# fchchen/omni-recall-rag

Measured on AMD Instinct MI355X. Metric: queries/sec at top-k=10 over N x 3072-d chunks; score delta vs C# reference in `parity`, higher is better.
Workload: dtype i8 screen + f32*f32->f64 exact re-score; 1 GPU; C3: 10000000 chunks x 3072-d fp32 on one GPU, batch=256 queries per step, top-k=10, full hybrid (cosine+keyword+recency), candidate_limit=corpus; corpus_rows=10000000

## Files before the change

### omni-recall-rag_amd/csrc/orr_api.hip

```cpp
#include <hip/hip_runtime.h>

#include <algorithm>
#include <cmath>
#include <cstdarg>
#include <cstdio>
#include <chrono>
#include <pthread.h>
#include <dlfcn.h>
#include <atomic>
#include <condition_variable>
#include <functional>
#include <cstring>
#include <limits>
#include <mutex>
#include <shared_mutex>
#include <deque>
#include <new>
#include <numeric>
#include <string>
#include <string_view>
#include <thread>
#include <unordered_map>
#include <vector>

// ... 106 lines not shown

}

struct orr_index {
    int device = 0;
    int32_t dim = 0;
    int64_t row_base = 0;
    hipStream_t stream = nullptr;
    hipStream_t stream_kw = nullptr;
    hipStream_t stream_aux = nullptr;
    hipEvent_t ev_bm_clean = nullptr;
    bool bm_clean_pending = false;
    bool kw_counters_clean = false;
    const void *kw_counters_of[2] = {nullptr, nullptr};
    hipEvent_t ev_inputs = nullptr, ev_kw_done = nullptr, ev_main_ready = nullptr, ev_range[15] = {};
    std::mutex mu;

    int64_t n_rows = 0, cap_rows = 0;
    float *d_emb = nullptr;
    int64_t *d_created = nullptr;
    int64_t *d_row_ids = nullptr;
    uint64_t *d_cstart = nullptr;
    uint32_t *d_clen = nullptr;
    uint8_t *d_pool = nullptr;
    uint64_t pool_len = 0, pool_cap = 0;
    double *d_norm_b = nullptr;
    int64_t n_tokens = 0;
    uint8_t *d_vpool = nullptr;
    uint64_t *d_vstart = nullptr;
    uint32_t *d_vlen = nullptr;
// ... 428 lines not shown
    HIP_TRY(hipGetDeviceProperties(&prop, cfg->device));
    if (strncmp(prop.gcnArchName, "gfx950", 6) != 0)
        return fail(ORR_EDEVICE, "device %d is %s; this library carries gfx950 code only", cfg->device, prop.gcnArchName);
    orr_index *idx = new (std::nothrow) orr_index();
    if (!idx) return fail(ORR_ENOMEM, "out of host memory");
    idx->device = cfg->device;
    idx->dim = cfg->dim;
    idx->row_base = cfg->row_base;
    if (hipSetDevice(idx->device) != hipSuccess || hipStreamCreateWithFlags(&idx->stream, hipStreamNonBlocking) != hipSuccess ||
        hipStreamCreateWithFlags(&idx->stream_kw, hipStreamNonBlocking) != hipSuccess ||
        hipStreamCreateWithFlags(&idx->stream_aux, hipStreamNonBlocking) != hipSuccess ||
        hipEventCreateWithFlags(&idx->ev_bm_clean, hipEventDisableTiming) != hipSuccess ||
        hipEventCreateWithFlags(&idx->ev_inputs, hipEventDisableTiming) != hipSuccess ||
        hipEventCreateWithFlags(&idx->ev_kw_done, hipEventDisableTiming) != hipSuccess ||
        hipEventCreateWithFlags(&idx->ev_main_ready, hipEventDisableTiming) != hipSuccess ||
        !create_range_events(idx->ev_range) ||
        hipEventCreateWithFlags(&idx->ev_q, hipEventDisableTiming) != hipSuccess) {
        orr_index_destroy(idx);
        return fail(ORR_EDEVICE, "cannot create streams on device %d", cfg->device);
    }
    if (cfg->capacity_rows > 0) {
        int r = ensure_row_capacity(idx, cfg->capacity_rows);
        if (r != ORR_OK) { orr_index_destroy(idx); return r; }
    }
    *out = idx;
    return ORR_OK;
}

void orr_index_destroy(orr_index *idx)
{
// ... 5 lines not shown
            LanePool::Exclusive all(&idx->lanes);
            views = idx->lanes.drain();
            idx->lanes.set_max_lanes(1);
        }
        for (orr_index *l : views) orr_index_destroy(l);
    }
    (void)hipSetDevice(idx->device);
    if (idx->stream) (void)hipStreamSynchronize(idx->stream);
    if (idx->stream_kw) (void)hipStreamSynchronize(idx->stream_kw);
    if (idx->stream_aux) (void)hipStreamSynchronize(idx->stream_aux);
    if (idx->ev_bm_clean) (void)hipEventDestroy(idx->ev_bm_clean);
    if (idx->stream_aux) (void)hipStreamDestroy(idx->stream_aux);
    if (idx->ev_inputs) (void)hipEventDestroy(idx->ev_inputs);
    if (idx->ev_kw_done) (void)hipEventDestroy(idx->ev_kw_done);
    if (idx->ev_main_ready) (void)hipEventDestroy(idx->ev_main_ready);
    for (hipEvent_t e : idx->ev_range) if (e) (void)hipEventDestroy(e);
    if (idx->stream_kw) (void)hipStreamDestroy(idx->stream_kw);
    for (auto &pe : idx->pending) { (void)hipEventDestroy(pe.start); (void)hipEventDestroy(pe.stop); }
    for (auto e : idx->event_pool) (void)hipEventDestroy(e);
    if (!idx->is_view) {
        if (idx->d_emb) (void)hipFree(idx->d_emb);
        if (idx->d_created) (void)hipFree(idx->d_created);
        if (idx->d_row_ids) (void)hipFree(idx->d_row_ids);
        if (idx->d_cstart) (void)hipFree(idx->d_cstart);
        if (idx->d_clen) (void)hipFree(idx->d_clen);
        if (idx->d_pool) (void)hipFree(idx->d_pool);
        if (idx->d_norm_b) (void)hipFree(idx->d_norm_b);
        if (idx->d_vpool) (void)hipFree(idx->d_vpool);
        if (idx->d_vstart) (void)hipFree(idx->d_vstart);
        if (idx->d_vlen) (void)hipFree(idx->d_vlen);
// ... 1309 lines not shown
    v->device = parent->device; v->dim = parent->dim; v->row_base = parent->row_base;
    v->n_rows = parent->n_rows; v->cap_rows = parent->cap_rows;
    v->d_emb = parent->d_emb; v->d_created = parent->d_created; v->d_row_ids = parent->d_row_ids; v->d_norm_b = parent->d_norm_b;
    v->n_tokens = parent->n_tokens; v->d_vpool = parent->d_vpool; v->d_vstart = parent->d_vstart; v->d_vlen = parent->d_vlen;
    v->d_post_off = parent->d_post_off; v->d_post_rows = parent->d_post_rows; v->n_postings = parent->n_postings;
    v->sealed = true;
    copy_options(parent, v);
    borrow_shadows(parent, v);
    if (hipStreamCreateWithFlags(&v->stream, hipStreamNonBlocking) != hipSuccess ||
        hipStreamCreateWithFlags(&v->stream_kw, hipStreamNonBlocking) != hipSuccess ||
        hipStreamCreateWithFlags(&v->stream_aux, hipStreamNonBlocking) != hipSuccess ||
        hipEventCreateWithFlags(&v->ev_bm_clean, hipEventDisableTiming) != hipSuccess ||
        hipEventCreateWithFlags(&v->ev_inputs, hipEventDisableTiming) != hipSuccess ||
        hipEventCreateWithFlags(&v->ev_kw_done, hipEventDisableTiming) != hipSuccess ||
        hipEventCreateWithFlags(&v->ev_main_ready, hipEventDisableTiming) != hipSuccess ||
        !create_range_events(v->ev_range) ||
        hipEventCreateWithFlags(&v->ev_q, hipEventDisableTiming) != hipSuccess) {
        v->internal_lane = true;
        orr_index_destroy(v);
        return fail(ORR_EDEVICE, "cannot create streams on device %d", parent->device);
    }
    v->internal_lane = internal;
    if (!internal) parent->user_views.fetch_add(1);
    *out = v;
    return ORR_OK;
}

int orr_index_screen_dots(orr_index *idx, int32_t B, int32_t dim, const float *q, float *out)
{
    if (!idx || !q || !out || B <= 0) return fail(ORR_EINVAL, "orr_index_screen_dots: bad argument");
// ... 32 lines not shown
    if (dim != idx->dim || dim <= 0 || dim % 128 != 0) return fail(ORR_EINVAL, "orr_index_screen_i8_dots: dim must equal the index dimension and be a multiple of 128");
    if (form > 0 && dim / 64 <= 6) return fail(ORR_EINVAL, "orr_index_screen_i8_dots: the four-wave forms need dim >= 448");
    if (idx->n_rows <= 0) return ORR_OK;
    HIP_TRY(hipSetDevice(idx->device));
    ORR_TRY(ensure_i8_shadow(idx));
    if (!idx->i8_ready) return fail(ORR_ENOMEM, "orr_index_screen_i8_dots: the int8 shadow does not fit in device memory");
    hipStream_t s = idx->stream;
    const size_t n = (size_t)idx->n_rows;
    ORR_TRY(idx->ws_q.reserve(sizeof(float) * (size_t)B * dim));
    ORR_TRY(idx->ws_q8.reserve(2 * (size_t)B * dim));
    ORR_TRY(idx->ws_q8s1.reserve(sizeof(float) * (size_t)B));
    ORR_TRY(idx->ws_q8err.reserve(2 * sizeof(double) * (size_t)B));
    ORR_TRY(idx->ws_qtiled.reserve(orr::i8_tiled_bytes(B, dim)));
    HIP_TRY(hipMemcpyAsync(idx->ws_q.p, q, sizeof(float) * (size_t)B * dim, hipMemcpyDefault, s));
    HIP_TRY(orr::launch_i8_queries(idx->ws_q.as<float>(), B, dim, idx->ws_q8.p, idx->ws_q8s1.as<float>(), idx->ws_q8err.as<double>(), s,
                                   idx->ws_q8err.as<double>() + B));
    HIP_TRY(orr::launch_i8_tile_queries(idx->ws_q8.p, B, dim, idx->ws_qtiled.p, s));
    if (out_dots) {
        ORR_TRY(idx->ws_dotf.reserve(sizeof(int32_t) * (size_t)B * n));
        HIP_TRY(hipMemsetAsync(idx->ws_dotf.p, 0xAB, sizeof(int32_t) * (size_t)B * n, s));
        ORR_TRY(idx->ws_tickets.reserve(sizeof(uint32_t) * 8 * 16));
        HIP_TRY(hipMemsetAsync(idx->ws_tickets.p, 0, sizeof(uint32_t) * 8 * 16, s));
        {
            Timed t(idx, form == 0 ? "screen_i8_dots_w8" : form == 1 ? "screen_i8_dots_w4" : "screen_i8_dots_w16",
                    1.0 * (double)n * dim + 1.0 * (double)B * dim + 4.0 * (double)B * (double)n);
            HIP_TRY(orr::launch_screen_i8_dots_raw(idx->ws_qtiled.p, B, idx->emb_i8.p, idx->n_rows, dim, idx->ws_dotf.as<int32_t>(),
                                                   idx->n_rows, form, nt_rows != 0, s, idx->ws_tickets.as<uint32_t>()));
        }
        HIP_TRY(hipMemcpyAsync(out_dots, idx->ws_dotf.p, sizeof(int32_t) * (size_t)B * n, hipMemcpyDefault, s));
    }
    if (out_iq) HIP_TRY(hipMemcpyAsync(out_iq, idx->ws_q8.p, (size_t)B * dim, hipMemcpyDefault, s));
    if (out_ie) {
// ... 217 lines not shown
        if (!on) return;
        const auto now = std::chrono::steady_clock::now();
        acc[i] += std::chrono::duration<double, std::milli>(now - last).count();
        last = now;
    }
    void done()
    {
        if (!on || ++calls % 64 != 0) return;
        fprintf(stderr, "[orr host ms/call] query_setup+cos_launch %.3f | keyword_prep+launch %.3f | norms+consts %.3f | select_launches %.3f | "
                        "wait_gpu %.3f | finish %.3f\n", acc[0] / 64, acc[1] / 64, acc[2] / 64, acc[3] / 64, acc[4] / 64, acc[5] / 64);
        for (double &x : acc) x = 0;
    }
};
thread_local HostTiming g_ht;

struct KwSide {
    orr::KwView view{nullptr, 0, nullptr, nullptr, nullptr};
    size_t bm_bytes = 0, bm_clean_before = 0;
    bool overflow_possible = false;
    uint32_t max_hits = 0;
    const uint8_t *alias = nullptr;
};

int launch_keyword_side(orr_index *idx, const BatchArgs &a, const std::vector<uint32_t> &qoff, KwSide &out)
{
    const int32_t B = a.B;
    const uint32_t t_begin = qoff[0], n_terms_total = qoff[(size_t)B] - qoff[0];
    if (n_terms_total == 0) return ORR_OK;
    {

        std::vector<std::string_view> dterms;
        dterms.reserve(n_terms_total);
        uint32_t table_size = 16;
        while (table_size < 2 * n_terms_total + 2) table_size <<= 1;
        std::vector<uint32_t> table(table_size, 0xFFFFFFFFu);
        std::vector<uint32_t> qmeta((size_t)n_terms_total + (size_t)B + 1);
// ... 183 lines not shown
            {
                Timed t(idx, "expand_hits", 0.0, k);
                HIP_TRY(orr::launch_expand_hits(idx->ws_hits.as<orr::KwHit>(), idx->ws_counter.as<unsigned long long>(), max_hits,
                                                idx->d_post_rows, idx->ws_bitmaps.as<uint32_t>(), words, k,
                                                idx->pin_kwcnt.as<unsigned long long>(), skip));
            }
        }
        ORR_TRY(settle_bitmaps());
        HIP_TRY(hipEventRecord(idx->ev_kw_done, k));
        out.view.bitmaps = idx->ws_bitmaps.as<uint32_t>();
        out.view.words_per_term = words;
        out.view.q_term_idx = reinterpret_cast<const uint32_t *>(dm + off_qmeta);
        out.view.q_term_off = out.view.q_term_idx + n_terms_total;
        out.overflow_possible = want_hits > (uint64_t)max_hits;
        out.max_hits = max_hits;
    }
    return ORR_OK;
}

int run_large_k(orr_index *idx, const BatchArgs &a, int32_t kprime, int64_t n, const double *d_dot, const orr::KwView &kw,
                const orr::QueryConst *qc, orr_candidate *d_cand, hipStream_t s)
{
    const int32_t B = a.B;
    ORR_TRY(idx->ws_keys_a.reserve(sizeof(unsigned long long) * (size_t)n));
    ORR_TRY(idx->ws_keys_b.reserve(sizeof(unsigned long long) * (size_t)n));
    ORR_TRY(idx->ws_vals_a.reserve(sizeof(uint32_t) * (size_t)n));
    ORR_TRY(idx->ws_vals_b.reserve(sizeof(uint32_t) * (size_t)n));
    size_t tmp_bytes = 0;
    HIP_TRY(orr::sort_pairs_desc(nullptr, tmp_bytes, idx->ws_keys_a.as<unsigned long long>(),
                                 idx->ws_keys_b.as<unsigned long long>(), idx->ws_vals_a.as<uint32_t>(),
// ... 197 lines not shown
    std::vector<int32_t> qgroup;
    uint32_t cap = 0;
    const uint32_t *d_qgroup = nullptr;
    const int64_t *d_took = nullptr;
    uint32_t *h_screened = nullptr;
};

struct PassIo {
    const float *d_q = nullptr;
    double *d_dot = nullptr;
    float *d_dotf = nullptr;
    orr::KwView kw{nullptr, 0, nullptr, nullptr, nullptr};
    const double2 *d_rowc = nullptr;
    orr_candidate *d_cand = nullptr;
    bool direct_host = false;
    const MaskScope *mask = nullptr;
    GroupScopes *groups = nullptr;
};

struct PassFront {
    std::vector<uint32_t> qoff;
    uint32_t n_terms_total = 0;
    size_t rec_bytes = 0;
    bool q_download_pending = false;
    PassIo io;
};

template <class Plan>
int open_pass(orr_index *idx, const BatchArgs &a, int32_t kprime, Plan &&plan, bool pinned_records, bool out_dev, bool dev_norms,
              const float **q_host, PassPlan &p, PassFront &f)
// ... 75 lines not shown
}

int launch_i8_query_image(orr_index *idx, const float *d_q, int32_t B, bool gemm, hipStream_t s)
{
    ORR_TRY(idx->ws_q8.reserve(2 * (size_t)B * idx->dim));
    ORR_TRY(idx->ws_q8s1.reserve(sizeof(float) * (size_t)B));
    if (!gemm) {
        ORR_TRY(idx->ws_q8err.reserve(sizeof(double) * (size_t)B));
        ORR_TRY(idx->ws_fcnt.reserve(sizeof(uint32_t) * 3 * (size_t)B));
        HIP_TRY(orr::launch_i8_queries(d_q, B, idx->dim, idx->ws_q8.p, idx->ws_q8s1.as<float>(), idx->ws_q8err.as<double>(), s, nullptr,
                                       idx->ws_fcnt.as<uint32_t>(), 3 * B));
        return ORR_OK;
    }
    ORR_TRY(idx->ws_q8err.reserve(2 * sizeof(double) * (size_t)B));
    ORR_TRY(idx->ws_qtiled.reserve(orr::i8_tiled_bytes(B, idx->dim)));
    HIP_TRY(orr::launch_i8_queries(d_q, B, idx->dim, idx->ws_q8.p, idx->ws_q8s1.as<float>(), idx->ws_q8err.as<double>(), s,
                                   idx->ws_q8err.as<double>() + B));
    HIP_TRY(orr::launch_i8_tile_queries(idx->ws_q8.p, B, idx->dim, idx->ws_qtiled.p, s));
    return ORR_OK;
}

int launch_numerators(orr_index *idx, const BatchArgs &a, const PassPlan &p, int64_t n, PassIo &io)
{
    if (!p.use_cos) return ORR_OK;
    const int32_t B = a.B;
    hipStream_t s = idx->stream;
    auto split_queries = [&]() -> int {
        ORR_TRY(idx->ws_qsplit.reserve(sizeof(float) * (size_t)B * idx->dim));
        HIP_TRY(orr::launch_split_queries(io.d_q, B, idx->dim, idx->ws_qsplit.p, s));
        return ORR_OK;
    };
    if (p.masked) {
        if (p.prefix_i8) return launch_i8_query_image(idx, io.d_q, B, true, s);
// ... 30 lines not shown
    ORR_TRY(idx->ws_dotf.reserve(sizeof(float) * (size_t)B * (size_t)dotf_rows));
    io.d_dotf = idx->ws_dotf.as<float>();
    if (p.prefix_i8) {
        ORR_TRY(launch_i8_query_image(idx, io.d_q, B, true, s));
        const int64_t pre_rows = std::min<int64_t>(dotf_rows, n);
        Timed t(idx, "screen_i8_prefix", 1.0 * (double)pre_rows * idx->dim + 1.0 * (double)B * idx->dim + 4.0 * (double)B * (double)pre_rows);
        HIP_TRY(orr::launch_screen_i8_dots(idx->ws_qtiled.p, B, idx->emb_i8.p, pre_rows, idx->dim, io.d_dotf, dotf_rows, s));
    } else {
        ORR_TRY(split_queries());
        Timed t(idx, "gemm_dot_bf16x3", 4.0 * (double)dotf_rows * idx->dim + 4.0 * (double)B * idx->dim + 4.0 * (double)B * (double)dotf_rows);
        HIP_TRY(orr::launch_gemm_dot_bf16x3(idx->ws_qsplit.p, B, idx->d_emb, 0, dotf_rows, idx->dim, io.d_dotf, dotf_rows, nullptr, 3, s));
    }
    return ORR_OK;
}

int launch_consts(orr_index *idx, const BatchArgs &a, const PassPlan &p, int64_t n, const std::vector<uint32_t> &qoff,
                  bool download_pending, PassIo &io)
{
    const int32_t B = a.B;
    hipStream_t s = idx->stream;
    if (download_pending) HIP_TRY(hipEventSynchronize(idx->ev_q));
    ORR_TRY(idx->pin_qc.reserve(sizeof(orr::QueryConst) * (size_t)B));
    ORR_TRY(idx->ws_qc.reserve(sizeof(orr::QueryConst) * (size_t)B));
    orr::QueryConst *qc = idx->pin_qc.as<orr::QueryConst>();
    if (p.use_cos && !p.dev_norms) {
        if (a.norms_host) memcpy(idx->h_norm_a.data(), a.norms_host, sizeof(double) * (size_t)B);
        else exact_norms(idx->pin_q.as<float>(), B, a.dim, idx->h_norm_a.data());
    }
    for (int32_t b = 0; b < B; ++b) {
        qc[b].use_cos = p.use_cos ? 1 : 0;
// ... 3 lines not shown
        qc[b].inv_sqrt_na = 0.0;
        if (p.batched_score && p.use_cos && !p.dev_norms) {
            if (qc[b].norm_a <= 0.0) qc[b].use_cos = 0;
            else qc[b].inv_sqrt_na = 1.0 / std::sqrt(qc[b].norm_a);
        }
    }
    if (p.dev_norms) {
        HIP_TRY(hipStreamWaitEvent(s, idx->ev_q, 0));
        HIP_TRY(orr::launch_patch_query_norms(idx->ws_qc.as<orr::QueryConst>(), idx->ws_norm_a.as<double>(), B, p.batched_score, s,
                                              idx->pin_norm.as<double>(), qc));
    } else {
        HIP_TRY(hipMemcpyAsync(idx->ws_qc.p, qc, sizeof(orr::QueryConst) * (size_t)B, hipMemcpyHostToDevice, s));
    }
    if (p.batched_score && !p.rowc_inline) {
        ORR_TRY(idx->ws_rowc.reserve(sizeof(double2) * (size_t)n));
        Timed t(idx, io.groups ? "row_consts_grouped" : io.mask ? "row_consts_masked" : "row_consts", 32.0 * (double)n);
        if (io.groups)
            HIP_TRY(orr::launch_row_consts_grouped(idx->d_norm_b, idx->d_created, a.now_ticks, n, io.groups->bm, io.groups->words,
                                                   io.groups->n_groups, io.groups->d_clip, idx->ws_rowc.as<double2>(), s));
        else if (io.mask)
            HIP_TRY(orr::launch_row_consts_masked(idx->d_norm_b, idx->d_created, a.now_ticks, n, io.mask->bm, idx->ws_rowc.as<double2>(), s));
        else
            HIP_TRY(orr::launch_row_consts(idx->d_norm_b, idx->d_created, a.now_ticks, n, idx->ws_rowc.as<double2>(), s));
        io.d_rowc = idx->ws_rowc.as<double2>();
    }
    return ORR_OK;
}

enum class Rescore {
    BufferExact,
    ScopeGeneric,
};

int rescore_survivors(orr_index *idx, const BatchArgs &a, const PassIo &io, const orr::FusedEpilogue &epi, uint32_t kCap, Rescore how,
                      double bytes, hipStream_t s)
{
    Timed t(idx, how == Rescore::BufferExact ? "rescore_buffer_exact" : "scope_rescore", bytes);
    HIP_TRY((how == Rescore::BufferExact ? orr::launch_rescore_buffer_exact : orr::launch_scope_rescore_generic)(
// ... 176 lines not shown
        }
        const bool gemm_i8 = p.screen == Screen::I8Ranges;
        if (gemm_i8) {
            epi.i8_rowf = idx->i8_rowf.as<float4>();
            epi.i8_qs1 = idx->ws_q8s1.as<float>();
        }
        HIP_TRY(orr::launch_fused_query_consts(idx->ws_qc.as<orr::QueryConst>(), idx->ws_tskey.as<unsigned long long>(), B,
                                               idx->ws_fqf.as<float4>(), s, gemm_i8 ? idx->ws_q8s1.as<float>() : nullptr,
                                               gemm_i8 ? idx->ws_q8err.as<double>() + B : nullptr,
                                               gemm_i8 ? idx->ws_fqf.as<float4>() + B : nullptr,
                                               idx->ws_fcnt.as<uint32_t>(), 3 * B, idx->ws_tickets.as<uint32_t>(), 8 * 16));
        epi.qf16 = gemm_i8 ? idx->ws_fqf.as<float4>() + B : nullptr;
    }
    epi.tau = idx->ws_tskey.as<unsigned long long>();
    if (p.screen == Screen::I8Ranges) {
        ORR_TRY(screen_i8_in_ranges(idx, a, p, n, io.kw, epi, s));
    } else if (p.screen == Screen::GemvI8) {
        Timed t(idx, "screen_gemv_i8", 1.0 * (double)n * idx->dim + 28.0 * (double)n + 2.0 * (double)B * idx->dim);
        HIP_TRY(orr::launch_screen_gemv_i8(idx->ws_q8.p, idx->ws_q8s1.as<float>(), idx->ws_q8err.as<double>(), B, idx->emb_i8.p,
                                           idx->i8_scale.as<float>(), idx->i8_rel_err.as<float>(), idx->i8_rel_hat.as<float>(),
                                           io.mask ? nullptr : idx->d_norm_b, idx->d_created, a.now_ticks, n, idx->dim, epi, false, s));
    } else if (p.screen == Screen::GemvBf16) {
        Timed t(idx, "screen_gemv_bf16", 2.0 * (double)n * idx->dim + 2.0 * (double)B * idx->dim);
        HIP_TRY(orr::launch_screen_gemv_bf16(idx->ws_qsplit.p, B, idx->emb_shadow.p, n, idx->dim, epi, s));
    } else if (p.screen == Screen::Bf16Shadow) {
        ORR_TRY(idx->ws_qtiled.reserve(orr::bf16_tiled_bytes(B, idx->dim)));
        HIP_TRY(orr::launch_bf16_tiled(io.d_q, B, idx->dim, idx->ws_qtiled.p, s));
        Timed t(idx, "screen_bf16_fused", 2.0 * (double)n * idx->dim + 2.0 * (double)B * idx->dim);
        HIP_TRY(orr::launch_screen_bf16(idx->ws_qtiled.p, B, idx->emb_shadow.p, 0, n, idx->dim, nullptr, 0, &epi, s));
    } else {
// ... 119 lines not shown
        Timed t(idx, "select_final", (double)B * (double)n_seg * orr::kSelWidth * sizeof(orr::SelEntry));
        HIP_TRY(orr::launch_select_final(idx->ws_sel.as<orr::SelEntry>(), n_seg32, B, kprime, n, idx->row_base,
                                         io.d_dot, io.d_dotf, n, idx->d_norm_b, idx->d_created, idx->d_row_ids, io.kw,
                                         p.use_mfma ? 0 : 1, p.approx_eps, nullptr, nullptr, 0u, nullptr, io.d_cand, s));
    }
    if (p.use_mfma && !p.two_stage()) {
        Timed t(idx, "rescore_exact", (double)B * kprime * 4.0 * idx->dim);
        HIP_TRY(orr::launch_rescore_exact(idx->d_emb, idx->dim, io.d_q, B, kprime, idx->row_base, io.d_cand, s));
    }
    return ORR_OK;
}

int clean_keyword_side(orr_index *idx, const KwSide &kws, uint32_t n_terms_total)
{
    if (kws.bm_bytes) {
        if (kws.bm_bytes >= ((size_t)16 << 20)) {
            HIP_TRY(hipMemsetAsync(idx->ws_bitmaps.p, 0, kws.bm_bytes, idx->stream_aux));
            HIP_TRY(hipEventRecord(idx->ev_bm_clean, idx->stream_aux));
            idx->bm_clean_pending = true;
        } else {
            HIP_TRY(hipMemsetAsync(idx->ws_bitmaps.p, 0, kws.bm_bytes, idx->stream_kw));
        }
        idx->bitmaps_clean = std::max(kws.bm_bytes, kws.bm_clean_before);
    }
    if (n_terms_total > 0 && idx->ws_counter.p) {
        HIP_TRY(hipMemsetAsync(idx->ws_counter.p, 0, sizeof(unsigned long long), idx->stream_kw));
        if (idx->ws_kwalias.p) HIP_TRY(hipMemsetAsync(idx->ws_kwalias.p, 0, idx->ws_kwalias.cap, idx->stream_kw));
        idx->kw_counters_clean = true;
        idx->kw_counters_of[0] = idx->ws_counter.p;
        idx->kw_counters_of[1] = idx->ws_kwalias.p;
    }
// ... 47 lines not shown
    ORR_TRY(open_pass(idx, a, kprime, [&](const std::vector<uint32_t> &qoff, PassPlan &plan) { return plan_pass(idx, a, kprime, n, qoff, plan); },
                      host_records, true, true, q_host, p, f));
    PassIo &io = f.io;

    if (p.form == PassForm::Empty) {
        const std::vector<orr_candidate> empty = empty_records(B, kprime);
        if (io.direct_host) memcpy(io.d_cand, empty.data(), f.rec_bytes);
        else HIP_TRY(hipMemcpyAsync(io.d_cand, empty.data(), f.rec_bytes, hipMemcpyHostToDevice, s));
        HIP_TRY(hipStreamSynchronize(s));
        if (f.q_download_pending || p.dev_norms) HIP_TRY(hipEventSynchronize(idx->ev_q));
        if (recs_host && io.direct_host) *recs_host = io.d_cand;
        return ORR_OK;
    }

    if (p.screen == Screen::GemvI8) ORR_TRY(launch_i8_query_image(idx, io.d_q, B, false, s));

    KwSide kws;
    ORR_TRY(launch_keyword_side(idx, a, f.qoff, kws));
    io.kw = kws.view;
    g_ht.mark(1);

    ORR_TRY(launch_numerators(idx, a, p, n, io));
    g_ht.mark(0);

    ORR_TRY(launch_consts(idx, a, p, n, f.qoff, f.q_download_pending, io));
    if (f.n_terms_total > 0) HIP_TRY(hipStreamWaitEvent(s, idx->ev_kw_done, 0));
    g_ht.mark(2);

    ORR_TRY(launch_selection(idx, a, p, kprime, n, io, host_records, f.rec_bytes));

    if (!owner_of(idx)->dead.empty())
        HIP_TRY(orr::launch_mark_dead_records(io.d_cand, B, kprime, owner_of(idx)->d_dead.as<int64_t>(),
                                              (int32_t)owner_of(idx)->dead.size(), idx->row_base, s));
    if (host_records) ORR_TRY(records_to_host(idx, f, s));
    g_ht.mark(3);
    idx->sstats.pass_mode = p.pass_mode();

    const int r = finish_pass(idx, a, p, kws, f.n_terms_total);
    if (r != ORR_OK) return r;
    if (recs_host && io.direct_host) *recs_host = io.d_cand;
// ... 3983 lines not shown
```

### omni-recall-rag_amd/csrc/orr_kernels.h

```cpp
#pragma once

#include <hip/hip_runtime.h>
#include <stdint.h>

#include "../../include/omnirecall_hip.h"
#include "orr_layout.h"
#include "orr_scope_plan.h"
#include "orr_mask_plan.h"
#include "orr_scope_set_plan.h"
#include "orr_scope_terms_plan.h"
#include "orr_scope_near_plan.h"
#include "orr_range_plan.h"

#include <atomic>

namespace orr {

inline int current_device_ordinal()
{
    int d = 0;
    if (hipGetDevice(&d) != hipSuccess || d < 0) d = 0;
    return d;
}
template <auto KERNEL>
// ... 100 lines not shown
    return h & (uint32_t)(kVocabBloomBits - 1);
}
hipError_t launch_vocab_match_lookup(const uint8_t *vpool, const uint64_t *vstart, const uint32_t *vlen, int64_t n_tokens,
                                     const MatchTerm *terms, const uint32_t *lk, const uint32_t *keys, const uint32_t *tidx,
                                     const uint32_t *bloom, const uint64_t *post_off, unsigned long long *counter, KwHit *hits,
                                     uint32_t max_hits, hipStream_t s);
hipError_t launch_vocab_match_mid(const uint8_t *vpool, const uint64_t *starts, const uint32_t *lens, const uint32_t *ids, int64_t n_list,
                                  const MatchTerm8 *terms, int32_t n_terms, const uint64_t *post_off, unsigned long long *counter,
                                  KwHit *hits, uint32_t max_hits, hipStream_t s);
hipError_t launch_expand_hits(const KwHit *hits, const unsigned long long *counter, uint32_t max_hits,
                              const uint32_t *post_rows, uint32_t *bitmaps, int64_t words_per_term, hipStream_t s,
                              unsigned long long *counter_host = nullptr, const uint8_t *skip_term = nullptr);
hipError_t launch_kw_alias(const KwHit *hits, const unsigned long long *counter, uint32_t max_hits, int32_t n_terms,
                           const int32_t *tok_bm_index, int64_t bm_store_delta, int64_t words_per_term, uint32_t *term_cnt,
                           uint32_t *term_tok, int64_t *term_word_off, uint8_t *alias, hipStream_t s);

struct QueryConst {
    double norm_a;
    double inv_sqrt_na;
    double inv_n_terms;
    int32_t n_terms;
    int32_t use_cos;
};

hipError_t launch_patch_query_norms(QueryConst *qc, const double *norm_a, int32_t B, bool batched, hipStream_t s,
                                    double *norm_host = nullptr,
                                    const QueryConst *qc_host = nullptr);

hipError_t launch_row_consts(const double *norm_b, const int64_t *created, int64_t now_ticks, int64_t n_rows,
                             double2 *out, hipStream_t s);
// ... 45 lines not shown
                                     const float *i8_qs1 = nullptr, const double *i8_qerr2 = nullptr, float4 *qf16 = nullptr,
                                     uint32_t *zero_a = nullptr, int32_t n_a = 0, uint32_t *zero_b = nullptr, int32_t n_b = 0);
size_t bf16_tiled_bytes(int64_t n_rows, int32_t D);
hipError_t launch_bf16_tiled(const float *X, int64_t n_rows, int32_t D, void *out, hipStream_t s);
hipError_t launch_screen_bf16(const void *q_tiled, int32_t B, const void *e_shadow, int64_t row_first, int64_t n_rows,
                              int32_t D, float *S, int64_t s_stride, const FusedEpilogue *epi, hipStream_t s);
hipError_t launch_screen_gemv_bf16(const void *q_hi, int32_t B, const void *e_shadow, int64_t n_rows, int32_t D,
                                   const FusedEpilogue &epi, hipStream_t s);
size_t i8_tiled_bytes(int64_t n_rows, int32_t D);
hipError_t launch_i8_shadow(const float *E, const double *norm_b, int64_t n_rows, int32_t D, void *tiled, float *scale,
                            float *rel_err, float *rel_hat, hipStream_t s);
hipError_t launch_update_rows(const float *rows, const double *norms, const int64_t *pos, const int64_t *src, int64_t src_base,
                              int64_t n_targets, int32_t D, float *E, double *norm_b, void *i8_tiled, float *i8_scale, float *i8_rel_err,
                              float *i8_rel_hat, float4 *i8_rowf, void *bf16_tiled, hipStream_t s);
hipError_t launch_i8_queries(const float *Q, int32_t B, int32_t D, void *q12, float *s1, double *err2, hipStream_t s,
                             double *err2_level1 = nullptr, uint32_t *zero = nullptr, int32_t n_zero = 0);
bool screen_gemv_i8_prefix_makes_lists(int32_t D);
hipError_t launch_screen_gemv_i8(const void *q12, const float *s1, const double *err2, int32_t B, const void *tiled,
                                 const float *scale, const float *rel_err, const float *rel_hat, const double *norm_b,
                                 const int64_t *created, int64_t now_ticks, int64_t n_rows, int32_t D,
                                 const FusedEpilogue &epi, bool lower_bound, hipStream_t s);
hipError_t launch_screen_gemv_i8_dots(const void *q12, int32_t B, const void *tiled, int64_t n_rows, int32_t D, int32_t *S, bool fine,
                                      hipStream_t s);
hipError_t launch_i8_rowf(const float *scale, const float *rel_err, const float *rel_hat, int64_t n_rows, float4 *rowf, hipStream_t s);
hipError_t launch_i8_tile_queries(const void *q1_linear, int32_t B, int32_t D, void *tiled, hipStream_t s);
hipError_t launch_screen_i8(const void *q_tiled, int32_t B, const void *e_tiled, int64_t n_rows, int32_t D,
                            const FusedEpilogue &epi, hipStream_t s, int64_t row_first = 0);
hipError_t launch_screen_i8_dots(const void *q_tiled, int32_t B, const void *e_tiled, int64_t n_rows, int32_t D, float *S,
                                 int64_t s_stride, hipStream_t s);
hipError_t launch_screen_i8_dots_raw(const void *q_tiled, int32_t B, const void *e_tiled, int64_t n_rows, int32_t D, int32_t *S,
                                     int64_t s_stride, int32_t form, bool nt_rows, hipStream_t s, uint32_t *tickets = nullptr);
// ... 135 lines not shown
```

### omni-recall-rag_amd/csrc/orr_kernels.hip

```cpp
#include "orr_kernels.h"
#include "orr_device.h"

#include <hipcub/hipcub.hpp>

#include <cstdlib>

namespace orr {

__global__ __launch_bounds__(256) void row_consts_kernel(const double *__restrict__ norm_b,
                                                         const int64_t *__restrict__ created, int64_t now_ticks,
                                                         int64_t n_rows, double2 *__restrict__ out)
{
    for (int64_t r = (int64_t)blockIdx.x * blockDim.x + threadIdx.x; r < n_rows; r += (int64_t)gridDim.x * blockDim.x) {
        out[r] = row_consts_of(norm_b[r], created[r], now_ticks);
    }
}

__global__ void patch_query_norms_kernel(QueryConst *__restrict__ qc, const double *__restrict__ norm_a, int32_t B, int32_t batched,
                                         double *__restrict__ norm_host, const QueryConst *__restrict__ qc_host)
{
    const int32_t b = blockIdx.x * blockDim.x + threadIdx.x;
    if (b >= B) return;
    const double na = norm_a[b];
    QueryConst c = qc_host ? qc_host[b] : qc[b];
// ... 428 lines not shown
            for (int g = 0; g < 4; ++g) {
                const uint32_t row = rows4[g];
                const bool live = row != 0xFFFFFFFFu;
                const uint32_t word = row >> 5;
                uint32_t bits = live ? 1u << (row & 31) : 0u;
#pragma unroll
                for (int d = 1; d < 32; d <<= 1) {
                    const uint32_t ow = (uint32_t)__shfl_up((int)word, d, 64), ob = (uint32_t)__shfl_up((int)bits, d, 64);
                    if (lane >= d && ow == word) bits |= ob;
                }
                const uint32_t nw = (uint32_t)__shfl_down((int)word, 1, 64);
                if (live && (lane == 63 || nw != word)) atomicOr(&bm[word], bits);
            }
        }
    }
}

hipError_t launch_vocab_hits(const uint16_t *vmatch, int64_t n_tokens, int32_t n_terms, const uint32_t *token_ids,
                             const uint64_t *post_off, unsigned long long *counter, KwHit *hits, uint32_t max_hits, hipStream_t s)
{
    if (n_tokens <= 0 || n_terms <= 0) return hipSuccess;
    int64_t blocks = (n_tokens * (int64_t)n_terms + 255) / 256;
    if (blocks > 4096) blocks = 4096;
    hipLaunchKernelGGL(vocab_hits_kernel, dim3((unsigned)blocks), dim3(256), 0, s, vmatch, n_tokens, n_terms, token_ids, post_off,
                       counter, hits, max_hits);
    return hipGetLastError();
}

__global__ __launch_bounds__(256) void vocab_match_short_kernel(const uint8_t *__restrict__ vpool,
                                                                const uint64_t *__restrict__ vstart,
// ... 1732 lines not shown
```

### omni-recall-rag_amd/csrc/orr_screen.hip

```cpp
#include "orr_kernels.h"
#include "orr_device.h"
#include "orr_epilogue.h"

#include <algorithm>
#include <cstdio>
#include <vector>
#include <type_traits>
#include <cstdlib>

namespace orr {

namespace {

constexpr int kScBM = 256, kScBN = 256, kScBK = 32;
constexpr int kScImage = kScBM * kScBK * 2;
#ifndef ORR_SC_NA
#define ORR_SC_NA 3
#define ORR_SC_NB 5
#endif
constexpr int kScNA = ORR_SC_NA, kScNB = ORR_SC_NB;
constexpr int kScEpiBytes = 32768;
constexpr int kScEpiQueue = 7;
constexpr int kScLds = (kScNA + kScNB) * kScImage + kScEpiBytes;
static_assert(kScLds <= 160 * 1024, "the rings and the epilogue's region must fit a CU's LDS");
// ... 1138 lines not shown
        if (row >= n_rows) {
            for (int k = lane * 4; k < D; k += 256)
                *reinterpret_cast<uint32_t *>(dst + i8_tiled_off(k, rr)) = 0u;
            continue;
        }
        const I8Row q = i8_quantise_row(E + row * (int64_t)D, D, lane, rr, dst);
        if (lane == 0) {
            scale[row] = q.se;
            i8_rel_norms(q, norm_b[row], rel_err[row], rel_hat[row]);
        }
    }
}

__global__ __launch_bounds__(256) void i8_queries_kernel(const float *__restrict__ Qf, int32_t D, int8_t *__restrict__ q1, int8_t *__restrict__ q2,
                                                         float *__restrict__ s1_out, double *__restrict__ err2_out,
                                                         double *__restrict__ err2_l1_out, uint32_t *__restrict__ zero, int32_t n_zero)
{
    if (blockIdx.x == 0) for (int i = threadIdx.x; i < n_zero; i += 256) zero[i] = 0u;
    __shared__ float red_f[4];
    __shared__ double red_d[4], red_d1[4];
    const int b = blockIdx.x, tid = threadIdx.x, lane = tid & 63, wave = tid >> 6;
    const float *q = Qf + (int64_t)b * D;
    float mx = 0.f;
    bool bad = false;
    for (int k = tid; k < D; k += 256) { const float v = q[k]; mx = fmaxf(mx, fabsf(v)); bad = bad || !(fabsf(v) <= 3.4028234663852886e38f); }
#pragma unroll
    for (int d = 32; d > 0; d >>= 1) mx = fmaxf(mx, __shfl_xor(mx, d, 64));
    bad = __any(bad);
    if (lane == 0) red_f[wave] = (bad ? __builtin_huge_valf() : mx);
    __syncthreads();
    mx = fmaxf(fmaxf(red_f[0], red_f[1]), fmaxf(red_f[2], red_f[3]));
    const bool usable = mx > 0.f && mx <= 3.4028234663852886e38f;
    const float s1 = usable ? mx / 127.f : 0.f, s2 = s1 / 254.f;
    double e2 = 0.0, e1 = 0.0;
    for (int k = tid; k < D; k += 256) {
        const float v = q[k];
        int a = usable ? __float2int_rn(v / s1) : 0;
        a = a > 127 ? 127 : (a < -127 ? -127 : a);
        const double r = (double)v - (double)s1 * (double)a;
        e1 += usable ? r * r : (double)v * (double)v;
        int c2 = (usable && s2 > 0.f) ? __double2int_rn(r / (double)s2) : 0;
        c2 = c2 > 127 ? 127 : (c2 < -127 ? -127 : c2);
        const double dl = r - (double)s1 * ((double)c2 / 254.0);
        e2 += usable ? dl * dl : (double)v * (double)v;
        q1[(int64_t)b * D + k] = (int8_t)a;
        q2[(int64_t)b * D + k] = (int8_t)c2;
    }
#pragma unroll
    for (int d = 32; d > 0; d >>= 1) { e2 += __shfl_xor(e2, d, 64); e1 += __shfl_xor(e1, d, 64); }
    if (lane == 0) { red_d[wave] = e2; red_d1[wave] = e1; }
    __syncthreads();
    if (tid == 0) {
        s1_out[b] = s1;
        const double tot = red_d[0] + red_d[1] + red_d[2] + red_d[3];
        const double tot1 = red_d1[0] + red_d1[1] + red_d1[2] + red_d1[3];
        const bool bounded = mx <= 3.4028234663852886e38f && !(mx > 0.f && mx < kI8MinQueryMax);
        err2_out[b] = bounded ? tot * 1.000001 : __builtin_huge_val();
        if (err2_l1_out) err2_l1_out[b] = bounded ? tot1 * 1.000001 : __builtin_huge_val();
    }
}

// ... 375 lines not shown

hipError_t launch_update_rows(const float *rows, const double *norms, const int64_t *pos, const int64_t *src, int64_t src_base,
                              int64_t n_targets, int32_t D, float *E, double *norm_b, void *i8_tiled, float *i8_scale, float *i8_rel_err,
                              float *i8_rel_hat, float4 *i8_rowf, void *bf16_tiled, hipStream_t s)
{
    if (n_targets <= 0) return hipSuccess;
    if (D <= 0 || (i8_tiled && D % 128 != 0) || (bf16_tiled && D % 64 != 0)) return hipErrorInvalidValue;
    if (i8_tiled && (!i8_scale || !i8_rel_err || !i8_rel_hat || !i8_rowf)) return hipErrorInvalidValue;
    const int64_t blocks = std::min<int64_t>((n_targets + 3) / 4, 65536);
    hipLaunchKernelGGL(update_rows_kernel, dim3((unsigned)blocks), dim3(256), 0, s, rows, norms, pos, src, src_base, n_targets, D, E, norm_b,
                       static_cast<int8_t *>(i8_tiled), i8_scale, i8_rel_err, i8_rel_hat, i8_rowf, static_cast<__bf16 *>(bf16_tiled));
    return hipGetLastError();
}

hipError_t launch_i8_queries(const float *Q, int32_t B, int32_t D, void *q12, float *s1, double *err2, hipStream_t s, double *err2_level1,
                             uint32_t *zero, int32_t n_zero)
{
    if (B <= 0) return hipSuccess;
    int8_t *q1 = static_cast<int8_t *>(q12);
    hipLaunchKernelGGL(i8_queries_kernel, dim3((unsigned)B), dim3(256), 0, s, Q, D, q1, q1 + (size_t)B * D, s1, err2, err2_level1, zero, zero ? n_zero : 0);
    return hipGetLastError();
}

bool screen_gemv_i8_prefix_makes_lists(int32_t D) { return D % 1024 == 0; }

static void screen_gemv_i8_grid(int64_t n_rows, bool fine, int64_t &n_units, int64_t &blocks)
{
    const int64_t tiles = (n_rows + kScBN - 1) / kScBN;
    n_units = tiles * (fine ? 16 : 2);
    blocks = std::min<int64_t>((n_units + 3) / 4, 512);
}

hipError_t launch_screen_gemv_i8(const void *q12, const float *s1, const double *err2, int32_t B, const void *tiled,
                                 const float *scale, const float *rel_err, const float *rel_hat, const double *norm_b,
                                 const int64_t *created, int64_t now_ticks, int64_t n_rows, int32_t D,
// ... 146 lines not shown
```

Before: 31080 queries/s.

## Overlap front-end setup: fuse query tiling, split row consts, reorder launches

Folds the i8 query tiling into the query-quantization kernel, so the separate tile launch goes away. Computes the tail of the row constants on the aux stream behind an event, overlapping it with the main stream. Lets numerators (and optionally consts) launch before the keyword side, and clears only non-aliased term bitmaps with a dedicated kernel instead of a full memset. An env var restores the serial path. The cost is added stream and event dependencies and more complex ordering.

```diff
diff --git a/omni-recall-rag_amd/csrc/orr_api.hip b/omni-recall-rag_amd/csrc/orr_api.hip
--- a/omni-recall-rag_amd/csrc/orr_api.hip
+++ b/omni-recall-rag_amd/csrc/orr_api.hip
@@ -144,6 +144,7 @@
     bool kw_counters_clean = false;
     const void *kw_counters_of[2] = {nullptr, nullptr};
     hipEvent_t ev_inputs = nullptr, ev_kw_done = nullptr, ev_main_ready = nullptr, ev_range[15] = {};
+    hipEvent_t ev_rowc = nullptr;
     std::mutex mu;
 
     int64_t n_rows = 0, cap_rows = 0;
@@ -602,6 +603,7 @@
         hipEventCreateWithFlags(&idx->ev_inputs, hipEventDisableTiming) != hipSuccess ||
         hipEventCreateWithFlags(&idx->ev_kw_done, hipEventDisableTiming) != hipSuccess ||
         hipEventCreateWithFlags(&idx->ev_main_ready, hipEventDisableTiming) != hipSuccess ||
+        hipEventCreateWithFlags(&idx->ev_rowc, hipEventDisableTiming) != hipSuccess ||
         !create_range_events(idx->ev_range) ||
         hipEventCreateWithFlags(&idx->ev_q, hipEventDisableTiming) != hipSuccess) {
         orr_index_destroy(idx);
@@ -637,6 +639,7 @@
     if (idx->ev_inputs) (void)hipEventDestroy(idx->ev_inputs);
     if (idx->ev_kw_done) (void)hipEventDestroy(idx->ev_kw_done);
     if (idx->ev_main_ready) (void)hipEventDestroy(idx->ev_main_ready);
+    if (idx->ev_rowc) (void)hipEventDestroy(idx->ev_rowc);
     for (hipEvent_t e : idx->ev_range) if (e) (void)hipEventDestroy(e);
     if (idx->stream_kw) (void)hipStreamDestroy(idx->stream_kw);
     for (auto &pe : idx->pending) { (void)hipEventDestroy(pe.start); (void)hipEventDestroy(pe.stop); }
@@ -1976,6 +1979,7 @@
         hipEventCreateWithFlags(&v->ev_inputs, hipEventDisableTiming) != hipSuccess ||
         hipEventCreateWithFlags(&v->ev_kw_done, hipEventDisableTiming) != hipSuccess ||
         hipEventCreateWithFlags(&v->ev_main_ready, hipEventDisableTiming) != hipSuccess ||
+        hipEventCreateWithFlags(&v->ev_rowc, hipEventDisableTiming) != hipSuccess ||
         !create_range_events(v->ev_range) ||
         hipEventCreateWithFlags(&v->ev_q, hipEventDisableTiming) != hipSuccess) {
         v->internal_lane = true;
@@ -2038,8 +2042,7 @@
     ORR_TRY(idx->ws_qtiled.reserve(orr::i8_tiled_bytes(B, dim)));
     HIP_TRY(hipMemcpyAsync(idx->ws_q.p, q, sizeof(float) * (size_t)B * dim, hipMemcpyDefault, s));
     HIP_TRY(orr::launch_i8_queries(idx->ws_q.as<float>(), B, dim, idx->ws_q8.p, idx->ws_q8s1.as<float>(), idx->ws_q8err.as<double>(), s,
-                                   idx->ws_q8err.as<double>() + B));
-    HIP_TRY(orr::launch_i8_tile_queries(idx->ws_q8.p, B, dim, idx->ws_qtiled.p, s));
+                                   idx->ws_q8err.as<double>() + B, nullptr, 0, idx->ws_qtiled.p));
     if (out_dots) {
         ORR_TRY(idx->ws_dotf.reserve(sizeof(int32_t) * (size_t)B * n));
         HIP_TRY(hipMemsetAsync(idx->ws_dotf.p, 0xAB, sizeof(int32_t) * (size_t)B * n, s));
@@ -2287,12 +2290,16 @@
 };
 thread_local HostTiming g_ht;
 
+static int front_mode() { const char *e = getenv("ORR_FRONT_SERIAL"); return e ? atoi(e) : 0; }
+static bool front_serial() { return front_mode() == 1; }
+
 struct KwSide {
     orr::KwView view{nullptr, 0, nullptr, nullptr, nullptr};
     size_t bm_bytes = 0, bm_clean_before = 0;
     bool overflow_possible = false;
     uint32_t max_hits = 0;
     const uint8_t *alias = nullptr;
+    uint32_t n_distinct = 0;
 };
 
 int launch_keyword_side(orr_index *idx, const BatchArgs &a, const std::vector<uint32_t> &qoff, KwSide &out)
@@ -2506,6 +2513,7 @@
         out.view.q_term_off = out.view.q_term_idx + n_terms_total;
         out.overflow_possible = want_hits > (uint64_t)max_hits;
         out.max_hits = max_hits;
+        out.n_distinct = TT;
     }
     return ORR_OK;
 }
@@ -2733,6 +2741,7 @@
     const double2 *d_rowc = nullptr;
     orr_candidate *d_cand = nullptr;
     bool direct_host = false;
+    bool rowc_tail = false;
     const MaskScope *mask = nullptr;
     GroupScopes *groups = nullptr;
 };
@@ -2838,9 +2847,10 @@
     }
     ORR_TRY(idx->ws_q8err.reserve(2 * sizeof(double) * (size_t)B));
     ORR_TRY(idx->ws_qtiled.reserve(orr::i8_tiled_bytes(B, idx->dim)));
+    const bool one_launch = !front_serial();
     HIP_TRY(orr::launch_i8_queries(d_q, B, idx->dim, idx->ws_q8.p, idx->ws_q8s1.as<float>(), idx->ws_q8err.as<double>(), s,
-                                   idx->ws_q8err.as<double>() + B));
-    HIP_TRY(orr::launch_i8_tile_queries(idx->ws_q8.p, B, idx->dim, idx->ws_qtiled.p, s));
+                                   idx->ws_q8err.as<double>() + B, nullptr, 0, one_launch ? idx->ws_qtiled.p : nullptr));
+    if (!one_launch) HIP_TRY(orr::launch_i8_tile_queries(idx->ws_q8.p, B, idx->dim, idx->ws_qtiled.p, s));
     return ORR_OK;
 }
 
@@ -2901,6 +2911,20 @@
     return ORR_OK;
 }
 
+int launch_row_consts_tail(orr_index *idx, const BatchArgs &a, const PassPlan &p, int64_t n, PassIo &io)
+{
+    if (front_serial() || p.form != PassForm::TwoStageGemm || p.screen != Screen::I8Ranges || p.masked || !p.batched_score ||
+        p.rowc_inline || p.dotf_rows >= n)
+        return ORR_OK;
+    ORR_TRY(idx->ws_rowc.reserve(sizeof(double2) * (size_t)n));
+    const int64_t r0 = p.dotf_rows;
+    Timed t(idx, "row_consts", 32.0 * (double)(n - r0), idx->stream_aux);
+    HIP_TRY(orr::launch_row_consts(idx->d_norm_b + r0, idx->d_created + r0, a.now_ticks, n - r0, idx->ws_rowc.as<double2>() + r0, idx->stream_aux));
+    HIP_TRY(hipEventRecord(idx->ev_rowc, idx->stream_aux));
+    io.rowc_tail = true;
+    return ORR_OK;
+}
+
 int launch_consts(orr_index *idx, const BatchArgs &a, const PassPlan &p, int64_t n, const std::vector<uint32_t> &qoff,
                   bool download_pending, PassIo &io)
 {
@@ -2934,14 +2958,15 @@
     }
     if (p.batched_score && !p.rowc_inline) {
         ORR_TRY(idx->ws_rowc.reserve(sizeof(double2) * (size_t)n));
-        Timed t(idx, io.groups ? "row_consts_grouped" : io.mask ? "row_consts_masked" : "row_consts", 32.0 * (double)n);
+        const int64_t rowc_rows = io.rowc_tail ? p.dotf_rows : n;
+        Timed t(idx, io.groups ? "row_consts_grouped" : io.mask ? "row_consts_masked" : "row_consts", 32.0 * (double)rowc_rows);
         if (io.groups)
             HIP_TRY(orr::launch_row_consts_grouped(idx->d_norm_b, idx->d_created, a.now_ticks, n, io.groups->bm, io.groups->words,
                                                    io.groups->n_groups, io.groups->d_clip, idx->ws_rowc.as<double2>(), s));
         else if (io.mask)
             HIP_TRY(orr::launch_row_consts_masked(idx->d_norm_b, idx->d_created, a.now_ticks, n, io.mask->bm, idx->ws_rowc.as<double2>(), s));
         else
-            HIP_TRY(orr::launch_row_consts(idx->d_norm_b, idx->d_created, a.now_ticks, n, idx->ws_rowc.as<double2>(), s));
+            HIP_TRY(orr::launch_row_consts(idx->d_norm_b, idx->d_created, a.now_ticks, rowc_rows, idx->ws_rowc.as<double2>(), s));
         io.d_rowc = idx->ws_rowc.as<double2>();
     }
     return ORR_OK;
@@ -3148,6 +3173,7 @@
     }
     epi.tau = idx->ws_tskey.as<unsigned long long>();
     if (p.screen == Screen::I8Ranges) {
+        if (io.rowc_tail) HIP_TRY(hipStreamWaitEvent(s, idx->ev_rowc, 0));
         ORR_TRY(screen_i8_in_ranges(idx, a, p, n, io.kw, epi, s));
     } else if (p.screen == Screen::GemvI8) {
         Timed t(idx, "screen_gemv_i8", 1.0 * (double)n * idx->dim + 28.0 * (double)n + 2.0 * (double)B * idx->dim);
@@ -3297,7 +3323,10 @@
 int clean_keyword_side(orr_index *idx, const KwSide &kws, uint32_t n_terms_total)
 {
     if (kws.bm_bytes) {
-        if (kws.bm_bytes >= ((size_t)16 << 20)) {
+        if (kws.alias && !front_serial()) {
+            HIP_TRY(orr::launch_clear_term_bitmaps(idx->ws_bitmaps.as<uint32_t>(), kws.view.words_per_term, (int32_t)kws.n_distinct,
+                                                   kws.alias, idx->stream_kw));
+        } else if (kws.bm_bytes >= ((size_t)16 << 20)) {
             HIP_TRY(hipMemsetAsync(idx->ws_bitmaps.p, 0, kws.bm_bytes, idx->stream_aux));
             HIP_TRY(hipEventRecord(idx->ev_bm_clean, idx->stream_aux));
             idx->bm_clean_pending = true;
@@ -3375,16 +3404,30 @@
     }
 
     if (p.screen == Screen::GemvI8) ORR_TRY(launch_i8_query_image(idx, io.d_q, B, false, s));
+    ORR_TRY(launch_row_consts_tail(idx, a, p, n, io));
+    const int front = front_mode();
+    const bool queries_first = front != 1 && p.form == PassForm::TwoStageGemm && p.prefix_i8 && p.dev_norms && !f.q_download_pending;
+    const bool consts_first = queries_first && front == 2;
+    if (queries_first) {
+        ORR_TRY(launch_numerators(idx, a, p, n, io));
+        g_ht.mark(0);
+    }
+    if (consts_first) {
+        ORR_TRY(launch_consts(idx, a, p, n, f.qoff, false, io));
+        g_ht.mark(2);
+    }
 
     KwSide kws;
     ORR_TRY(launch_keyword_side(idx, a, f.qoff, kws));
     io.kw = kws.view;
     g_ht.mark(1);
 
-    ORR_TRY(launch_numerators(idx, a, p, n, io));
-    g_ht.mark(0);
-
-    ORR_TRY(launch_consts(idx, a, p, n, f.qoff, f.q_download_pending, io));
+    if (!queries_first) {
+        ORR_TRY(launch_numerators(idx, a, p, n, io));
+        g_ht.mark(0);
+    }
+
+    if (!consts_first) ORR_TRY(launch_consts(idx, a, p, n, f.qoff, f.q_download_pending, io));
     if (f.n_terms_total > 0) HIP_TRY(hipStreamWaitEvent(s, idx->ev_kw_done, 0));
     g_ht.mark(2);
 
diff --git a/omni-recall-rag_amd/csrc/orr_kernels.h b/omni-recall-rag_amd/csrc/orr_kernels.h
--- a/omni-recall-rag_amd/csrc/orr_kernels.h
+++ b/omni-recall-rag_amd/csrc/orr_kernels.h
@@ -138,6 +138,7 @@
 hipError_t launch_kw_alias(const KwHit *hits, const unsigned long long *counter, uint32_t max_hits, int32_t n_terms,
                            const int32_t *tok_bm_index, int64_t bm_store_delta, int64_t words_per_term, uint32_t *term_cnt,
                            uint32_t *term_tok, int64_t *term_word_off, uint8_t *alias, hipStream_t s);
+hipError_t launch_clear_term_bitmaps(uint32_t *bitmaps, int64_t words_per_term, int32_t n_terms, const uint8_t *alias, hipStream_t s);
 
 struct QueryConst {
     double norm_a;
@@ -213,7 +214,7 @@
                               int64_t n_targets, int32_t D, float *E, double *norm_b, void *i8_tiled, float *i8_scale, float *i8_rel_err,
                               float *i8_rel_hat, float4 *i8_rowf, void *bf16_tiled, hipStream_t s);
 hipError_t launch_i8_queries(const float *Q, int32_t B, int32_t D, void *q12, float *s1, double *err2, hipStream_t s,
-                             double *err2_level1 = nullptr, uint32_t *zero = nullptr, int32_t n_zero = 0);
+                             double *err2_level1 = nullptr, uint32_t *zero = nullptr, int32_t n_zero = 0, void *tiled = nullptr);
 bool screen_gemv_i8_prefix_makes_lists(int32_t D);
 hipError_t launch_screen_gemv_i8(const void *q12, const float *s1, const double *err2, int32_t B, const void *tiled,
                                  const float *scale, const float *rel_err, const float *rel_hat, const double *norm_b,
diff --git a/omni-recall-rag_amd/csrc/orr_kernels.hip b/omni-recall-rag_amd/csrc/orr_kernels.hip
--- a/omni-recall-rag_amd/csrc/orr_kernels.hip
+++ b/omni-recall-rag_amd/csrc/orr_kernels.hip
@@ -466,6 +466,33 @@
             }
         }
     }
+}
+
+constexpr int64_t kClearPiece = 2048;
+__global__ __launch_bounds__(256) void clear_term_bitmaps_kernel(uint4 *__restrict__ bitmaps, int64_t vec_per_term, int32_t n_terms,
+                                                                 const uint8_t *__restrict__ alias)
+{
+    const int64_t pieces = (vec_per_term + kClearPiece - 1) / kClearPiece;
+    const int64_t total = pieces * (int64_t)n_terms;
+    for (int64_t w = blockIdx.x; w < total; w += gridDim.x) {
+        const int64_t t = w / pieces;
+        if (alias[t]) continue;
+        const int64_t v0 = (w - t * pieces) * kClearPiece;
+        const int64_t v1 = v0 + kClearPiece < vec_per_term ? v0 + kClearPiece : vec_per_term;
+        uint4 *dst = bitmaps + t * vec_per_term;
+        for (int64_t v = v0 + threadIdx.x; v < v1; v += 256) dst[v] = make_uint4(0u, 0u, 0u, 0u);
+    }
+}
+
+hipError_t launch_clear_term_bitmaps(uint32_t *bitmaps, int64_t words_per_term, int32_t n_terms, const uint8_t *alias, hipStream_t s)
+{
+    if (n_terms <= 0 || words_per_term <= 0) return hipSuccess;
+    if (words_per_term % 4 != 0 || (reinterpret_cast<uintptr_t>(bitmaps) & 15u) != 0 || !alias) return hipErrorInvalidValue;
+    const int64_t vec = words_per_term / 4;
+    const int64_t total = (vec + kClearPiece - 1) / kClearPiece * (int64_t)n_terms;
+    hipLaunchKernelGGL(clear_term_bitmaps_kernel, dim3((unsigned)std::min<int64_t>(total, 8192)), dim3(256), 0, s,
+                       reinterpret_cast<uint4 *>(bitmaps), vec, n_terms, alias);
+    return hipGetLastError();
 }
 
 hipError_t launch_vocab_hits(const uint16_t *vmatch, int64_t n_tokens, int32_t n_terms, const uint32_t *token_ids,
diff --git a/omni-recall-rag_amd/csrc/orr_screen.hip b/omni-recall-rag_amd/csrc/orr_screen.hip
--- a/omni-recall-rag_amd/csrc/orr_screen.hip
+++ b/omni-recall-rag_amd/csrc/orr_screen.hip
@@ -1176,9 +1176,18 @@
 
 __global__ __launch_bounds__(256) void i8_queries_kernel(const float *__restrict__ Qf, int32_t D, int8_t *__restrict__ q1, int8_t *__restrict__ q2,
                                                          float *__restrict__ s1_out, double *__restrict__ err2_out,
-                                                         double *__restrict__ err2_l1_out, uint32_t *__restrict__ zero, int32_t n_zero)
+                                                         double *__restrict__ err2_l1_out, uint32_t *__restrict__ zero, int32_t n_zero,
+                                                         int8_t *__restrict__ tiled)
 {
     if (blockIdx.x == 0) for (int i = threadIdx.x; i < n_zero; i += 256) zero[i] = 0u;
+    int8_t *const trow = tiled ? tiled + (int64_t)(blockIdx.x >> 8) * kScBM * D + (int)(blockIdx.x & 255) * 64 : nullptr;
+    if (tiled) {
+        const int n_q = (int)gridDim.x, padded = (n_q + kScBM - 1) / kScBM * kScBM;
+        for (int p = n_q + (int)blockIdx.x; p < padded; p += n_q) {
+            int8_t *const dst = tiled + (int64_t)(p >> 8) * kScBM * D + (p & 255) * 64;
+            for (int k = threadIdx.x * 4; k < D; k += 1024) *reinterpret_cast<uint32_t *>(dst + i8_tiled_off(k, p & 255)) = 0u;
+        }
+    }
     __shared__ float red_f[4];
     __shared__ double red_d[4], red_d1[4];
     const int b = blockIdx.x, tid = threadIdx.x, lane = tid & 63, wave = tid >> 6;
@@ -1207,6 +1216,7 @@
         e2 += usable ? dl * dl : (double)v * (double)v;
         q1[(int64_t)b * D + k] = (int8_t)a;
         q2[(int64_t)b * D + k] = (int8_t)c2;
+        if (trow) trow[i8_tiled_off(k, b & 255)] = (int8_t)a;
     }
 #pragma unroll
     for (int d = 32; d > 0; d >>= 1) { e2 += __shfl_xor(e2, d, 64); e1 += __shfl_xor(e1, d, 64); }
@@ -1612,11 +1622,13 @@
 }
 
 hipError_t launch_i8_queries(const float *Q, int32_t B, int32_t D, void *q12, float *s1, double *err2, hipStream_t s, double *err2_level1,
-                             uint32_t *zero, int32_t n_zero)
+                             uint32_t *zero, int32_t n_zero, void *tiled)
 {
     if (B <= 0) return hipSuccess;
+    if (tiled && (D <= 0 || D % 128 != 0)) return hipErrorInvalidValue;
     int8_t *q1 = static_cast<int8_t *>(q12);
-    hipLaunchKernelGGL(i8_queries_kernel, dim3((unsigned)B), dim3(256), 0, s, Q, D, q1, q1 + (size_t)B * D, s1, err2, err2_level1, zero, zero ? n_zero : 0);
+    hipLaunchKernelGGL(i8_queries_kernel, dim3((unsigned)B), dim3(256), 0, s, Q, D, q1, q1 + (size_t)B * D, s1, err2, err2_level1, zero, zero ? n_zero : 0,
+                       static_cast<int8_t *>(tiled));
     return hipGetLastError();
 }
 
```

Result: faster. 31440 queries/s (median of 4 runs) (+1.2%).
